# mariusbaehr/gauss_newton_via_generalized_krylov_subspaces

Measured on NVIDIA B200. Metric: gnk_outer_iterations_per_second, higher is better.
Workload: dtype f64

## Files before the change

### gauss_newton_via_generalized_krylov_subspaces_b200/_lib.py

```python
from __future__ import annotations

import ctypes as C
import os

_HERE = os.path.dirname(os.path.abspath(__file__))
LIB_PATH = os.path.join(_HERE, "libgnk_b200.so")

GNK_MAX_BASIS = 256


class Layout(C.Structure):
    _fields_ = [("n_own", C.c_int64), ("off", C.c_int64), ("ld", C.c_int64), ("m", C.c_int32),
                ("rows", C.c_int32), ("halo", C.c_int32), ("has_lo", C.c_int32), ("has_hi", C.c_int32),
                ("pad_", C.c_int32)]


class Bratu(C.Structure):
    _fields_ = [("c_lap", C.c_double), ("c_adv", C.c_double), ("lam", C.c_double)]


class LinOp(C.Structure):
    _fields_ = [("kind", C.c_int32), ("pad_", C.c_int32), ("sign", C.c_double), ("lay", Layout), ("prm", Bratu),
                ("d_expu", C.c_void_p), ("n_res", C.c_int64), ("p", C.c_int64), ("d_rowptr", C.c_void_p),
                ("d_col", C.c_void_p), ("d_val", C.c_void_p), ("d_rowptr_t", C.c_void_p), ("d_col_t", C.c_void_p),
                ("d_val_t", C.c_void_p)]


_P = C.c_void_p
_I = C.c_int
_L = C.c_int64
_D = C.c_double
_LP = C.POINTER(Layout)
_BP = C.POINTER(Bratu)

SIGNATURES = {
    "gnk_abi_version": (_I, []),
    "gnk_last_error": (C.c_char_p, []),
    "gnk_create": (_I, [C.POINTER(_P), _I]),
    "gnk_destroy": (_I, [_P]),
    "gnk_sm_count": (_I, [_P]),
    "gnk_launch_count": (_L, [_P]),
    "gnk_scalars_fetch": (_I, [_P, _P, _I, _P, _P]),
    "gnk_scalars_wait": (_I, [_P]),
    "gnk_bratu_residual": (_I, [_P, _LP, _BP, _P, _P, _P, _P, _I, _P, _P]),
    "gnk_stencil_apply": (_I, [_P, _LP, _BP, _P, _P, _L, _I, _D, _I, _P, _L, _L, _P]),
    "gnk_stencil_normal_diag": (_I, [_P, _LP, _BP, _P, _P, _P]),
    "gnk_combine": (_I, [_P, _LP, _P, _I, _P, _P, _D, _P, _P]),
    "gnk_combine_step": (_I, [_P, _LP, _P, _I, _P, _P, _D, _P, _P, _P, _P]),
    "gnk_norm_stats": (_I, [_P, _LP, _P, _P, _P]),
    "gnk_normalize": (_I, [_P, _LP, _P, _P, _D, _P, _P, _P]),
    "gnk_normalize_halo": (_I, [_P, _LP, _P, _P, _D, _P, _P, _P]),
    "gnk_cgs_dots": (_I, [_P, _LP, _P, _I, _P, _P, _P]),
    "gnk_cgs_update": (_I, [_P, _LP, _P, _I, _P, _P, _P, _P]),
    "gnk_tsqr_ls": (_I, [_P, _P, _L, _L, _I, _P, _D, _P, _P]),
    "gnk_stencil_gram_ls": (_I, [_P, _LP, _BP, _P, _P, _L, _I, _I, _P, _D, _P, _L, _D, _P, _P]),
    "gnk_tsqr_ls_method": (_I, [_P, _I]),
    "gnk_gram_cgls": (_I, [_P, _P, _L, _L, _I, _P, _D, _D, _P, _P]),
    "gnk_spmm_csr": (_I, [_P, _L, _P, _P, _P, _P, _L, _L, _I, _D, _P, _L, _L, _P]),
    "gnk_csr_row_sumsq": (_I, [_P, _L, _P, _P, _P, _P]),
    "gnk_axpby": (_I, [_P, _L, _D, _P, _D, _P, _P, _P]),
    "gnk_dot": (_I, [_P, _L, _P, _P, _P, _P]),
    "gnk_cgls": (_I, [_P, C.POINTER(LinOp), _P, _D, _I, _P, _P, C.POINTER(_L), _P]),
    "gnk_cgls_x0": (_I, [_P, C.POINTER(LinOp), _P, _P, _D, _I, _P, _P, C.POINTER(_L), _P]),
    "gnk_rosenbrock_residual": (_I, [_P, _L, _D, _P, _P, _P]),
    "gnk_rosenbrock_jacobian": (_I, [_P, _L, _D, _P, _P, _P, _P]),
    "gnk_comm_unique_id": (_I, [_P]),
    "gnk_comm_init": (_I, [_P, _P, _I, _I]),
    "gnk_comm_size": (_I, [_P]),
    "gnk_comm_p2p_export": (_I, [_P, _P]),
    "gnk_comm_p2p_attach": (_I, [_P, _P]),
    "gnk_comm_p2p_enabled": (_I, [_P]),
    "gnk_comm_p2p_disable": (_I, [_P]),
    "gnk_comm_fused_reductions": (_I, [_P]),
    "gnk_comm_allreduce": (_I, [_P, _P, _I, _I, _P]),
    "gnk_comm_halo_exchange": (_I, [_P, _LP, _P, _I, _P]),
    "gnk_comm_allgather_owned": (_I, [_P, _LP, _P, _P, C.POINTER(_L), _P]),
}


class GnkError(RuntimeError):
    pass


_lib = None


def load():
    global _lib
# ... 37 lines not shown
```

### gauss_newton_via_generalized_krylov_subspaces_b200/csrc/bratu_stencil.cu

```cuda
#include "common.cuh"

namespace {

constexpr int TPBX = 128;

template <bool VEC>
struct Pair {
  double a, b;
};

template <bool VEC>
__device__ __forceinline__ Pair<VEC> load_pair(const double* p) {
  Pair<VEC> r;
  if (VEC) {
    double2 v = *reinterpret_cast<const double2*>(p);
    r.a = v.x;
    r.b = v.y;
  } else {
    r.a = *p;
    r.b = 0.0;
  }
  return r;
}
template <bool VEC>
// ... 103 lines not shown
  const int rend = min(rbeg + TR, lay.rows);
  const double* vb = in + (int64_t)col * in_ld + lay.off + j0;
  const double* eb_ = expu ? expu + lay.off + j0 : nullptr;
  double* ob = out + (int64_t)col * out_ld + out_off + j0;
  const bool has_l = j0 > 0, has_r = (j0 + W) < m;
  const double d0 = __dadd_rn(4.0 * prm.c_lap, -prm.c_adv);
  const double c_sup = __dadd_rn(-prm.c_lap, prm.c_adv);
  const double cu = transpose ? c_sup : -prm.c_lap;
  const double cd = transpose ? -prm.c_lap : c_sup;
  const double cl = -prm.c_lap;
  Pair<VEC> up = load_pair<VEC>(vb + (int64_t)(rbeg - 1) * m);
  Pair<VEC> mid = load_pair<VEC>(vb + (int64_t)rbeg * m);
#pragma unroll 2
  for (int r = rbeg; r < rend; ++r) {
    const int64_t ro = (int64_t)r * m;
    Pair<VEC> dn = load_pair<VEC>(vb + ro + m);
    const double lf = has_l ? vb[ro - 1] : 0.0;
    const double rt = has_r ? vb[ro + W] : 0.0;
    double dga = d0, dgb = d0;
    if (eb_) {
      Pair<VEC> e = load_pair<VEC>(eb_ + ro);
      dga = __dadd_rn(d0, __dmul_rn(prm.lam, e.a));
      dgb = __dadd_rn(d0, __dmul_rn(prm.lam, e.b));
    }
    const double ra = VEC ? mid.b : rt;
    const double oa = apply_refbits(cu, cl, dga, cd, up.a, lf, mid.a, ra, dn.a);
    const double ob2 = VEC ? apply_refbits(cu, cl, dgb, cd, up.b, mid.a, mid.b, rt, dn.b) : 0.0;
    store_pair<VEC>(ob + ro, sign * oa, sign * ob2);
    up = mid;
    mid = dn;
  }
}

template <bool VEC>
__global__ void __launch_bounds__(TPBX) normal_diag_kernel(gnk_layout lay, gnk_bratu prm,
                                                            const double* __restrict__ expu, int TR,
                                                            double* __restrict__ out) {
  constexpr int W = VEC ? 2 : 1;
  const int m = lay.m;
  const int j0 = W * (blockIdx.x * TPBX + threadIdx.x);
  if (j0 >= m) return;
  const int rbeg = (int)blockIdx.y * TR;
  const int rend = min(rbeg + TR, lay.rows);
  const double d0 = 4.0 * prm.c_lap - prm.c_adv;
  const double cl2 = prm.c_lap * prm.c_lap;
  const double cd2 = (prm.c_adv - prm.c_lap) * (prm.c_adv - prm.c_lap);
  for (int r = rbeg; r < rend; ++r) {
    const int64_t ro = lay.off + (int64_t)r * m + j0;
    double dga = d0, dgb = d0;
    if (expu) {
      Pair<VEC> e = load_pair<VEC>(expu + ro);
      dga = fma(prm.lam, e.a, d0);
      dgb = fma(prm.lam, e.b, d0);
    }
    const bool above = (r > 0) || lay.has_lo;
    const bool below = (r < lay.rows - 1) || lay.has_hi;
    double base = (above ? cd2 : 0.0) + (below ? cl2 : 0.0);
    double a = dga * dga + base + ((j0 > 0) ? cl2 : 0.0) + ((j0 + 1 < m) ? cl2 : 0.0);
    double b = 0.0;
    if (VEC) b = dgb * dgb + base + cl2 + ((j0 + 2 < m) ? cl2 : 0.0);
    store_pair<VEC>(out + ro, a, b);
  }
}


inline int pick_tr(const gnk_ctx* ctx, int gx, int rows, int mult) {
// ... 47 lines not shown
  if (vec)
    GNK_CUDA(gnk_launch(gnk_pdl_for(lay->n_own), residual_kernel<true>, grid, dim3(TPBX), 0, (cudaStream_t)stream, *lay, *prm, d_u, d_y, d_F, d_expu,
                        depth, tr, part, ctx->d_tickets + TK_RESID, d_loss, pd));
  else
    GNK_CUDA(gnk_launch(gnk_pdl_for(lay->n_own), residual_kernel<false>, grid, dim3(TPBX), 0, (cudaStream_t)stream, *lay, *prm, d_u, d_y, d_F,
                        d_expu, depth, tr, part, ctx->d_tickets + TK_RESID, d_loss, pd));
  GNK_LAUNCH_CHECK(ctx);
  return 0;
}

int gnk_stencil_apply(gnk_ctx* ctx, const gnk_layout* lay, const gnk_bratu* prm, const double* d_expu,
                      const double* d_in, int64_t in_ld, int k, double sign, int transpose, double* d_out,
                      int64_t out_ld, int64_t out_off, void* stream) {
  GNK_REQUIRE(ctx && prm && d_in && d_out, "gnk_stencil_apply: null argument");
  GNK_REQUIRE(check_layout(lay) == 0, "gnk_stencil_apply: inconsistent stencil layout");
  GNK_REQUIRE(k >= 1 && k <= 65535, "gnk_stencil_apply: k out of range");
  GNK_REQUIRE(prm->lam == 0.0 || d_expu, "gnk_stencil_apply: e^u diagonal required when lam != 0");
  const bool vec = (lay->m % 2) == 0 && (in_ld % 2) == 0 && (out_ld % 2) == 0 && (out_off % 2) == 0;
  const int gx = (int)ceil_div(lay->m, (vec ? 2 : 1) * TPBX);
  const int tr = pick_tr(ctx, gx, lay->rows, k);
  dim3 grid(k, gx, (unsigned)ceil_div(lay->rows, tr));
  GNK_REQUIRE(grid.z <= 65535, "gnk_stencil_apply: too many row tiles");
  const double* e = (prm->lam == 0.0) ? nullptr : d_expu;
  if (vec)
    GNK_CUDA(gnk_launch(gnk_pdl_for(lay->n_own), apply_kernel<true>, grid, dim3(TPBX), 0, (cudaStream_t)stream, *lay, *prm, e, d_in, in_ld, sign,
                        transpose, tr, d_out, out_ld, out_off));
  else
    GNK_CUDA(gnk_launch(gnk_pdl_for(lay->n_own), apply_kernel<false>, grid, dim3(TPBX), 0, (cudaStream_t)stream, *lay, *prm, e, d_in, in_ld, sign,
                        transpose, tr, d_out, out_ld, out_off));
  GNK_LAUNCH_CHECK(ctx);
  return 0;
}

int gnk_stencil_normal_diag(gnk_ctx* ctx, const gnk_layout* lay, const gnk_bratu* prm, const double* d_expu,
                            double* d_out, void* stream) {
  GNK_REQUIRE(ctx && prm && d_out, "gnk_stencil_normal_diag: null argument");
  GNK_REQUIRE(check_layout(lay) == 0, "gnk_stencil_normal_diag: inconsistent stencil layout");
  GNK_REQUIRE(prm->lam == 0.0 || d_expu, "gnk_stencil_normal_diag: e^u diagonal required when lam != 0");
  const bool vec = (lay->m % 2) == 0;
  const int gx = (int)ceil_div(lay->m, (vec ? 2 : 1) * TPBX);
  const int tr = pick_tr(ctx, gx, lay->rows, 1);
  dim3 grid(gx, (unsigned)ceil_div(lay->rows, tr));
  const double* e = (prm->lam == 0.0) ? nullptr : d_expu;
  if (vec)
    normal_diag_kernel<true><<<grid, TPBX, 0, (cudaStream_t)stream>>>(*lay, *prm, e, tr, d_out);
  else
    normal_diag_kernel<false><<<grid, TPBX, 0, (cudaStream_t)stream>>>(*lay, *prm, e, tr, d_out);
  GNK_LAUNCH_CHECK(ctx);
  return 0;
}

}
```

### gauss_newton_via_generalized_krylov_subspaces_b200/csrc/common.cuh

```cuda
#pragma once
#include <cuda_runtime.h>
#include <stdint.h>
#include <stdio.h>
#include <string>

#include "gnk_b200.h"

struct gnk_ctx {
  int device = 0;
  int sm_count = 148;
  int64_t launches = 0;
  double* d_partials = nullptr;
  unsigned int* d_tickets = nullptr;
  double* d_rbuf[2] = {nullptr, nullptr};
  size_t rbuf_bytes = 0;
  void* nccl_comm = nullptr;
  int rank = 0, nranks = 1;
  double* d_gather = nullptr;
  size_t gather_bytes = 0;
  double* h_pinned = nullptr;
  void* p2p_local = nullptr;
  void* p2p_peer[16] = {nullptr};
  void** d_p2p_peer = nullptr;
  unsigned long long p2p_seq = 0;
  unsigned long long p2p_hseq = 0;
  int p2p_ready = 0;
  int p2p_fused = 0;
  double* d_apart = nullptr;
  size_t apart_bytes = 0;
  double* d_cholqr = nullptr;
  double* d_gramw = nullptr;
  int ls_method = 0;
  cudaStream_t fetch_stream = nullptr;
  cudaEvent_t fetch_event = nullptr;
  cudaEvent_t cg_event[4] = {nullptr, nullptr, nullptr, nullptr};
};
int gnk_ensure_fetch_stream(gnk_ctx* ctx);

constexpr int GNK_PARTIALS = 1 << 19;
constexpr int GNK_TICKETS = 64;

constexpr int64_t PART_STATS = 0;
constexpr int64_t PART_DOTS = 8192;
constexpr int64_t PART_UPDATE = PART_DOTS + 1184 * GNK_MAX_BASIS;
constexpr int64_t PART_DOT1 = PART_UPDATE + 8192;
constexpr int64_t PART_CG = PART_DOT1 + 8192;
constexpr int64_t PART_SCAL = PART_CG + 8192;
constexpr int64_t PART_RESID = GNK_PARTIALS - 65536;
static_assert(PART_SCAL + 64 <= PART_RESID, "partials scratch overflow");

enum TicketSlot { TK_RESID = 0, TK_STATS = 1, TK_DOTS = 2, TK_UPDATE = 3, TK_DOT1 = 4, TK_CG = 5, TK_APPLY_DOTS = 6,
                  TK_CHOLQR = 7, TK_NORMALIZE = 8, TK_GRAMW = 9 };

void gnk_set_error(const std::string& s);
int gnk_fail(const char* what, cudaError_t e, const char* file, int line);

#define GNK_CUDA(expr)                                                    \
  do {                                                                    \
    cudaError_t e__ = (expr);                                             \
    if (e__ != cudaSuccess) return gnk_fail(#expr, e__, __FILE__, __LINE__); \
  } while (0)

#define GNK_LAUNCH_CHECK(ctx)                                             \
  do {                                                                    \
    (ctx)->launches++;                                                    \
    cudaError_t e__ = cudaGetLastError();                                 \
    if (e__ != cudaSuccess) return gnk_fail("kernel launch", e__, __FILE__, __LINE__); \
  } while (0)

#define GNK_REQUIRE(cond, msg)                                            \
  do {                                                                    \
    if (!(cond)) {                                                        \
      gnk_set_error(std::string(msg) + " (" #cond ")");                   \
      return -2;                                                          \
    }                                                                     \
  } while (0)

__device__ __forceinline__ double warp_sum(double v) {
#pragma unroll
  for (int o = 16; o > 0; o >>= 1) v += __shfl_xor_sync(0xffffffffu, v, o);
  return v;
}
__device__ __forceinline__ double warp_max(double v) {
#pragma unroll
  for (int o = 16; o > 0; o >>= 1) v = fmax(v, __shfl_xor_sync(0xffffffffu, v, o));
// ... 117 lines not shown
      asm volatile("ld.volatile.global.v4.u32 {%0, %1, %2, %3}, [%4];" : "=r"(lo), "=r"(t1), "=r"(hi), "=r"(t2) : "l"(p) : "memory");
      if (global_ns() - t0 > P2P_TIMEOUT_NS) __trap();
    } while (t1 != tag || t2 != tag);
  }
  return __hiloint2double((int)hi, (int)lo);
}
__device__ __forceinline__ void p2p_tail_allreduce(const gnk_p2p_dev& pd, double* vals, int count, int op) {
  const int t = threadIdx.x;
  if (t >= count) return;
  const int parity = (int)(pd.seq & 1ull);
  const unsigned tag = (unsigned)(pd.seq % 0xFFFFFFFFull) + 1u;
  const double v = vals[t];
  for (int r = 0; r < pd.nranks; ++r)
    st_ll(static_cast<char*>(pd.peers[r]) + p2p_ll_off(pd.nranks, parity, pd.rank) + 16 * (size_t)t, v, tag);
  const char* mine = static_cast<const char*>(pd.peers[pd.rank]);
  const bool is_max = (op == 1) || (op == 2 && t == 1);
  double a = ld_ll(mine + p2p_ll_off(pd.nranks, parity, 0) + 16 * (size_t)t, tag);
  for (int r = 1; r < pd.nranks; ++r) {
    const double b = ld_ll(mine + p2p_ll_off(pd.nranks, parity, r) + 16 * (size_t)t, tag);
    a = is_max ? fmax(a, b) : a + b;
  }
  vals[t] = a;
}

__device__ __forceinline__ double apply_refbits(double cu, double cl, double dg, double cd, double up, double lf,
                                                double mid, double rt, double dn) {
  double s = __dadd_rn(__dmul_rn(cu, up), __dmul_rn(cl, lf));
  s = __dadd_rn(s, __dmul_rn(dg, mid));
  s = __dadd_rn(s, __dmul_rn(cl, rt));
  s = __dadd_rn(s, __dmul_rn(cd, dn));
  return s;
}

static inline int64_t ceil_div(int64_t a, int64_t b) { return (a + b - 1) / b; }

__device__ __forceinline__ void pdl_begin() {
  asm volatile("griddepcontrol.wait;" ::: "memory");
  asm volatile("griddepcontrol.launch_dependents;" ::: "memory");
}
int gnk_pdl_mode();
constexpr int64_t GNK_PDL_MAX_N = 6 * 1024 * 1024;
inline bool gnk_pdl_for(int64_t n_unknowns) {
  const int mode = gnk_pdl_mode();
  return mode == 2 || (mode == 1 && n_unknowns <= GNK_PDL_MAX_N);
}
template <typename... P, typename... A>
inline cudaError_t gnk_launch(bool pdl, void (*kern)(P...), dim3 grid, dim3 block, size_t smem, cudaStream_t st,
                              A&&... args) {
  cudaLaunchConfig_t cfg = {};
  cfg.gridDim = grid;
  cfg.blockDim = block;
  cfg.dynamicSmemBytes = smem;
  cfg.stream = st;
  cudaLaunchAttribute at[1];
  at[0].id = cudaLaunchAttributeProgrammaticStreamSerialization;
  at[0].val.programmaticStreamSerializationAllowed = pdl ? 1 : 0;
  cfg.attrs = at;
  cfg.numAttrs = 1;
  return cudaLaunchKernelEx(&cfg, kern, static_cast<P>(args)...);
}
```

### gauss_newton_via_generalized_krylov_subspaces_b200/csrc/vector_ops.cu

```cuda
#include "common.cuh"

namespace {

constexpr int TPB = 256;

__device__ __forceinline__ double2 ld2(const double* p) { return *reinterpret_cast<const double2*>(p); }
__device__ __forceinline__ double2 ld2_stream(const double* p) {
  return __ldcs(reinterpret_cast<const double2*>(p));
}
__device__ __forceinline__ void st2(double* p, double2 v) { *reinterpret_cast<double2*>(p) = v; }

__global__ void __launch_bounds__(TPB) combine_kernel(const double* __restrict__ V, int64_t ld, int64_t len,
                                                       int k, const double* __restrict__ c,
                                                       const double* __restrict__ d, double s,
                                                       double* __restrict__ x, double* __restrict__ c_out,
                                                       double* __restrict__ cprev2) {
  __shared__ double coef[GNK_MAX_BASIS];
  pdl_begin();
  for (int j = threadIdx.x; j < k; j += blockDim.x) coef[j] = d ? (c[j] + s * d[j]) : c[j];
  __syncthreads();
  if (blockIdx.x == 0) {
    if (c_out) {
      for (int j = threadIdx.x; j <= k && j < GNK_MAX_BASIS; j += blockDim.x) c_out[j] = (j < k) ? coef[j] : 0.0;
    }
    if (cprev2 && threadIdx.x < 32) {
      double a = 0.0;
      for (int j = threadIdx.x; j < k; j += 32) a = fma(c[j], c[j], a);
      a = warp_sum(a);
      if (threadIdx.x == 0) cprev2[0] = a;
    }
  }
  const int64_t nv = len >> 1;
  const int64_t stride = (int64_t)gridDim.x * blockDim.x;
  for (int64_t i = (int64_t)blockIdx.x * blockDim.x + threadIdx.x; i < nv; i += stride) {
    const double* p = V + 2 * i;
    double2 acc = make_double2(0.0, 0.0);
    int j = 0;
    for (; j + 8 <= k; j += 8) {
      double2 v[8];
#pragma unroll
      for (int u = 0; u < 8; ++u) v[u] = ld2_stream(p + (int64_t)(j + u) * ld);
#pragma unroll
      for (int u = 0; u < 8; ++u) {
        acc.x = fma(v[u].x, coef[j + u], acc.x);
        acc.y = fma(v[u].y, coef[j + u], acc.y);
      }
    }
    for (; j < k; ++j) {
      double2 v = ld2_stream(p + (int64_t)j * ld);
      acc.x = fma(v.x, coef[j], acc.x);
      acc.y = fma(v.y, coef[j], acc.y);
    }
    st2(x + 2 * i, acc);
  }
}

__global__ void __launch_bounds__(TPB) stats_kernel(const double* __restrict__ x, int64_t n,
                                                     double* __restrict__ partials, unsigned int* ticket,
                                                     double* __restrict__ out) {
  __shared__ double sh[32];
  const int64_t nv = n >> 1;
  const int64_t gt = (int64_t)blockIdx.x * blockDim.x + threadIdx.x;
  const int64_t stride = (int64_t)gridDim.x * blockDim.x;
  double ss = 0.0, mx = 0.0;
// ... 418 lines not shown
```

### gauss_newton_via_generalized_krylov_subspaces_b200/gauss_newton_krylow.py

```python
from __future__ import annotations

import ctypes as C
import os
import weakref
from typing import Any, Callable, Optional, Tuple

import numpy as np

from . import _lib
from .armijo_goldstein import armijo_device
from .bratu_pde_problem import BratuDeviceProblem
from .device import DeviceVector, HostCallableProblem, get_runtime, make_layout, ptr
from .krylow import (GeneralizedKrylowSubspace, GeneralizedKrylowSubspaceBreakdown,
                     GeneralizedKrylowSubspaceSpansEntireSpace, MAX_COLUMNS)
from .partition import flat_layout_fields, round_up, tensor_ls_on_every_rank
from .regression_result import RegressionResult
from .rosenbrock_problem import RosenbrockDeviceProblem

_NB = _lib.GNK_MAX_BASIS
_SC_LOSS = 2 * _NB + 8
_SC_CPREV = _SC_LOSS + 2
_SC_FLAG = _SC_CPREV + 2
_SC_FLAG2 = _SC_CPREV + 3
_BLK = _SC_CPREV + 6
# ... 192 lines not shown
        r0 = np.asarray(res(prob.download_global(x_trial), *args), dtype=np.float64).reshape(-1)
        prob._ensure_res_layout(r0.shape[0])
    F_cur, F_trial = prob.new_res(), prob.new_res()
    res_off = prob.res_fields["off"]
    n_res_own = prob.res_fields["n_own"]
    ldjv = round_up(max(n_res_own, 1), 16)
    use_aux = is_bratu and prob.pb.LAMBDA != 0
    aux = [prob.new_sol() for _ in range(3)] if use_aux else [None, None, None]
    hx = prob.d.halo_exchange if (is_bratu and prob.distributed) else None
    ls_method = 0
    if is_bratu and prob.distributed and not tensor_ls_on_every_rank(prob.sol_fields["m"], rt.world):
        ls_method = 1

    if native:
        prob.residual(x_trial, F_cur, loss_slot, aux=None)
    else:
        rt.upload(r0, F_cur[:n_res_own])
        prob.sumsq(F_cur, loss_slot, prob.res_lay)
    nfev = 1
    prev_loss = float(rt.read(loss_slot, 1)[0])
    jac_ev = prob.jacobian(x_start, aux=None)
    if use_aux:
        aux[0] = jac_ev.expu
    njev = 1

    JV = None
    jv_cap = 0
    state = {"pending": False, "fslot": _SC_FLAG}

    def other_slot():
        return _SC_FLAG2 if state["fslot"] == _SC_FLAG else _SC_FLAG

    defer_ok = ls_solver == "qr" and os.environ.get("GNK_DEFER_BREAKDOWN", "1") != "0"

    for iter in range(1, max_iter):
        for attempt in (0, 1):
            k = krylow.k
            state["rank_reported"] = False
            if k > jv_cap:
                jv_cap = min(MAX_COLUMNS, max(krylow.cap, k))
                JV = rt.empty(jv_cap * ldjv)
            ls_done = False
            if (is_bratu and ls_solver == "qr" and ls_method == 0 and not jac_ev.transposed
                    and jac_ev.scale == 1.0):
                with rt.mark("spmm+ls", 8.0 * n_res_own * (3 * k + 2)) as mk:
                    rc = lib.gnk_stencil_gram_ls(rt.ctx, C.byref(sol_lay), C.byref(prob.d.prm), ptr(jac_ev.expu),
                                                 ptr(krylow.V), ld, krylow.cap, k, ptr(F_cur), -1.0, ptr(JV), ldjv,
                                                 -1.0, ptr(blk), rt.stream)
                    mk.cancel = rc != 0
                if rc == 0:
                    ls_done = True
                elif rc != 1:
                    _lib.check(rc, "gnk_stencil_gram_ls")
            if not ls_done:
                with rt.mark("spmm", 8.0 * n_res_own * (2 * k + 1)):
                    jac_ev.matmat(krylow.V, ld, k, JV, ldjv)
            if ls_done:
                pass
            elif ls_solver == "qr":
                with rt.mark("tsqr", 8.0 * n_res_own * (k + 1)):
                    tsqr_solve(rt, JV, ldjv, n_res_own, k, F_cur[res_off:], -1.0, blk, method=ls_method)
            elif ls_solver == "cgls":
                if k + 1 <= 56 and n_res_own % 2 == 0 and ldjv % 2 == 0:
                    with rt.mark("gram_cgls", 8.0 * n_res_own * (k + 1)):
                        _lib.check(lib.gnk_gram_cgls(rt.ctx, ptr(JV), ldjv, n_res_own, k, ptr(F_cur, res_off), -1.0,
                                                     float(cg_rtol), ptr(blk), rt.stream), "gnk_gram_cgls")
                else:
                    cgls_dense(rt, JV, ldjv, n_res_own, k, F_cur[res_off:], -1.0, cg_rtol, blk)
            else:
                raise ValueError("ls_solver must be 'qr' or 'cgls'")
            spec_ok = (native and defer_ok and iter + 1 < max_iter and iter % krylow_restart != 0
                       and version in _VERSIONS and krylow.k < prob.p_glob
                       and os.environ.get("GNK_SPECULATE", "1") != "0")
            state["spec"] = None

            def expansion_operands(jac_new):
                if version == "res_old":
                    return jac_new, F_cur
                if version == "res_new":
                    return jac_new, F_trial
                if version == "jac_old_res_old":
                    return jac_ev, F_cur
                return jac_ev, F_trial

            def trial_loss(s):
                krylow.dev_combine(c, blk, s, x_trial, c_out=c_next, cprev2=ptr(blk, _SC_CPREV))
                with rt.mark("residual", 32.0 * n_res_own):
                    prob.residual(x_trial, F_trial, loss_slot, aux=aux[1])
                if spec_ok and state["spec"] is None:
                    pending_read = rt.read_begin(blk, _BLK)
                    jac_new = prob.jacobian(x_trial, aux=aux[1])
                    krylow.dev_expand_enqueue(*expansion_operands(jac_new), hx, ptr(blk, other_slot()))
                    state["spec"] = jac_new
                    state["vals"] = rt.read_end(pending_read)
                else:
                    if state["spec"] is not None:
                        state["spec"] = False
                    state["vals"] = rt.read(blk, _BLK)
                if state["pending"] and state["vals"][state["fslot"]:state["fslot"] + 1].view(np.int32)[0] != 0:
                    raise _DeferredBreakdown()
                if ls_solver == "qr" and ls_refused(state["vals"], k):
                    raise _LeastSquaresRefused()
                if ls_solver == "qr" and not state["rank_reported"]:
                    state["rank_reported"] = True
                    _report_rank(state["vals"], k)
                return float(state["vals"][_SC_LOSS])

            def line_search():
                return armijo_device(trial_loss, prev_loss, lambda: float(state["vals"][k]),
                                     lambda: float(np.sqrt(state["vals"][k + 3])))

            try:
                step_length, nfev_delta = line_search()
            except _DeferredBreakdown:
                state["pending"] = False
                krylow.retract()
                print(f"Generalized krylow subspace breakdown at iteration = {iter - 1}, "
                      f"basis.shape = ({prob.p_glob}, {krylow.k})")
                continue
            except _LeastSquaresRefused:
                with rt.mark("tsqr", 8.0 * n_res_own * (k + 1)):
                    tsqr_solve(rt, JV, ldjv, n_res_own, k, F_cur[res_off:], -1.0, blk, householder=True)
                state["rank_reported"] = False
                step_length, nfev_delta = line_search()
            state["pending"] = False
# ... 69 lines not shown
```

### gauss_newton_via_generalized_krylov_subspaces_b200/krylow.py

```python
from __future__ import annotations

import ctypes as C
import math

import numpy as np

from . import _lib
from .device import CsrJacobian, HostCallableProblem, get_runtime, make_layout, ptr
from .partition import flat_layout_fields

MAX_COLUMNS = _lib.GNK_MAX_BASIS - 1


class GeneralizedKrylowSubspaceBreakdown(Exception):
    pass


class GeneralizedKrylowSubspaceSpansEntireSpace(Exception):
    pass


class _FlatOwner:

    def __init__(self, rt, n):
# ... 28 lines not shown
        self.flag = rt.zeros(1, dtype=rt.torch.int32)
        self._ready = True

    def _grow(self):
        if self.cap >= MAX_COLUMNS:
            raise _lib.GnkError(f"Krylov basis wider than {MAX_COLUMNS} columns is not supported; pass krylow_restart")
        new_cap = min(MAX_COLUMNS, max(self.cap * 2, 2), self.n_glob)
        V = self.rt.empty(new_cap * self.ld)
        V[:self.k * self.ld].copy_(self.V[:self.k * self.ld])
        self.V, self.cap = V, new_cap

    def col(self, j):
        return self.V[j * self.ld:(j + 1) * self.ld]

    def dev_start(self, x):
        rt, lib = self.rt, self.rt.lib
        _lib.check(lib.gnk_norm_stats(rt.ctx, C.byref(self.lay), ptr(x), ptr(self.stats), rt.stream), "gnk_norm_stats")
        rt.allreduce(self.stats, 2, 2)
        _lib.check(lib.gnk_normalize(rt.ctx, C.byref(self.lay), ptr(x), ptr(self.stats), 1e-8, ptr(self.V),
                                     ptr(self.flag), rt.stream), "gnk_normalize")
        ss = rt.read(self.stats, 2)
        if ss[1] <= 1e-8:
            raise ValueError("x0 is not allowed to be 0 in the gauss_newton_krylow algorithm")
        self.k = 1
        return math.sqrt(ss[0])

    def dev_combine(self, c, d, s, out, c_out=None, cprev2=None):
        rt = self.rt
        with rt.mark("combine", 8.0 * self.fields["n_own"] * (self.k + 1)):
            _lib.check(rt.lib.gnk_combine_step(rt.ctx, C.byref(self.lay), ptr(self.V), self.k, ptr(c), ptr(d), float(s),
                                               ptr(out), ptr(c_out), cprev2 if cprev2 is not None else ptr(None),
                                               rt.stream), "gnk_combine")

    def dev_expand_enqueue(self, jac_op, r, halo_exchange=None, flag_ptr=None):
        if self.k == self.n_glob:
            raise GeneralizedKrylowSubspaceSpansEntireSpace
        rt, lib = self.rt, self.rt.lib
        if self.k == self.cap:
            self._grow()
        n = self.fields["n_own"]
        with rt.mark("spmv_t", 24.0 * n):
            jac_op.neg_rmatvec(r, self.w)
        for ipass in range(self.reorth_passes):
            with rt.mark("cgs_dots", 8.0 * n * (self.k + 1)):
                _lib.check(lib.gnk_cgs_dots(rt.ctx, C.byref(self.lay), ptr(self.V), self.k, ptr(self.w),
                                            ptr(self.h), rt.stream), "gnk_cgs_dots")
            if not rt.fused_reductions:
                rt.allreduce(self.h, self.k, 0)
            with rt.mark("cgs_update", 8.0 * n * (self.k + 2)):
                _lib.check(lib.gnk_cgs_update(rt.ctx, C.byref(self.lay), ptr(self.V), self.k, ptr(self.h),
                                              ptr(self.w), ptr(self.stats), rt.stream), "gnk_cgs_update")
        if not rt.fused_reductions:
            rt.allreduce(self.stats, 2, 2)
        new = self.col(self.k)
        fp = ptr(self.flag) if flag_ptr is None else flag_ptr
        with rt.mark("normalize", 16.0 * n):
            if halo_exchange is not None:
                _lib.check(lib.gnk_normalize_halo(rt.ctx, C.byref(self.lay), ptr(self.w), ptr(self.stats), 1e-8,
                                                  ptr(new), fp, rt.stream), "gnk_normalize_halo")
            else:
                _lib.check(lib.gnk_normalize(rt.ctx, C.byref(self.lay), ptr(self.w), ptr(self.stats), 1e-8, ptr(new),
                                             fp, rt.stream), "gnk_normalize")

    def commit(self):
        self.k += 1

    def dev_update(self, jac_op, r, halo_exchange=None, deferred_flag=None):
        self.dev_expand_enqueue(jac_op, r, halo_exchange, deferred_flag)
        if deferred_flag is None and int(self.rt.read_i32(self.flag)[0]) != 0:
            raise GeneralizedKrylowSubspaceBreakdown(
                "Normal residual is allready inside generalized Krylow Subspcae, there for gauss newton krylow "
                "algorithm has to proceed without enlarging the subspace.")
        self.commit()

    def retract(self):
        self.k -= 1

    @property
    def basis(self):
        cols = [self.owner.download_global(self.col(j)) for j in range(self.k)]
        return np.stack(cols, axis=1)
# ... 47 lines not shown
```

### include/gnk_b200.h

```cpp
#ifndef GNK_B200_H
#define GNK_B200_H

#include <stdint.h>

#ifdef __cplusplus
extern "C" {
#endif

#define GNK_B200_ABI_VERSION 1
#define GNK_MAX_BASIS 256
#define GNK_TSQR_MAX 104

typedef struct gnk_ctx gnk_ctx;

typedef struct {
  int64_t n_own;
  int64_t off;
  int64_t ld;
  int32_t m;
  int32_t rows;
  int32_t halo;
  int32_t has_lo;
  int32_t has_hi;
  int32_t pad_;
// ... 7 lines not shown

int gnk_abi_version(void);
const char* gnk_last_error(void);
int gnk_create(gnk_ctx** out, int device);
int gnk_destroy(gnk_ctx* ctx);
int gnk_sm_count(gnk_ctx* ctx);
int64_t gnk_launch_count(gnk_ctx* ctx);
int gnk_scalars_fetch(gnk_ctx* ctx, const double* d_src, int count, double* h_dst, void* stream);
int gnk_scalars_wait(gnk_ctx* ctx);

int gnk_bratu_residual(gnk_ctx* ctx, const gnk_layout* lay, const gnk_bratu* prm, const double* d_u,
                       const double* d_y, double* d_F, double* d_expu, int depth, double* d_loss,
                       void* stream);
int gnk_stencil_apply(gnk_ctx* ctx, const gnk_layout* lay, const gnk_bratu* prm, const double* d_expu,
                      const double* d_in, int64_t in_ld, int k, double sign, int transpose,
                      double* d_out, int64_t out_ld, int64_t out_off, void* stream);
int gnk_stencil_normal_diag(gnk_ctx* ctx, const gnk_layout* lay, const gnk_bratu* prm,
                            const double* d_expu, double* d_out, void* stream);

int gnk_combine(gnk_ctx* ctx, const gnk_layout* lay, const double* d_V, int k, const double* d_c,
                const double* d_d, double s, double* d_x, void* stream);
int gnk_combine_step(gnk_ctx* ctx, const gnk_layout* lay, const double* d_V, int k, const double* d_c,
                     const double* d_d, double s, double* d_x, double* d_c_out, double* d_cprev2, void* stream);
int gnk_norm_stats(gnk_ctx* ctx, const gnk_layout* lay, const double* d_x, double* d_stats, void* stream);
int gnk_normalize(gnk_ctx* ctx, const gnk_layout* lay, const double* d_x, const double* d_stats,
                  double atol, double* d_out, int32_t* d_flag, void* stream);
int gnk_normalize_halo(gnk_ctx* ctx, const gnk_layout* lay, const double* d_x, const double* d_stats, double atol,
                       double* d_out, int32_t* d_flag, void* stream);
int gnk_cgs_dots(gnk_ctx* ctx, const gnk_layout* lay, const double* d_V, int k, const double* d_w,
                 double* d_h, void* stream);
int gnk_cgs_update(gnk_ctx* ctx, const gnk_layout* lay, const double* d_V, int k, const double* d_h,
                   double* d_w, double* d_stats, void* stream);

int gnk_tsqr_ls(gnk_ctx* ctx, const double* d_A, int64_t lda, int64_t n_rows, int k,
                const double* d_y, double sign_a, double* d_out, void* stream);

int gnk_stencil_gram_ls(gnk_ctx* ctx, const gnk_layout* lay, const gnk_bratu* prm, const double* d_expu,
                        const double* d_V, int64_t ldv, int v_cols, int k, const double* d_r, double sign,
                        double* d_JV, int64_t ldjv, double sign_a, double* d_out, void* stream);

int gnk_tsqr_ls_method(gnk_ctx* ctx, int method);

int gnk_spmm_csr(gnk_ctx* ctx, int64_t n_rows, const int32_t* d_rowptr, const int32_t* d_col,
                 const double* d_val, const double* d_in, int64_t in_ld, int64_t in_off, int k,
                 double sign, double* d_out, int64_t out_ld, int64_t out_off, void* stream);
int gnk_csr_row_sumsq(gnk_ctx* ctx, int64_t n_rows, const int32_t* d_rowptr, const double* d_val,
                      double* d_out, void* stream);

int gnk_axpby(gnk_ctx* ctx, int64_t n, double a, const double* d_x, double b, const double* d_y,
              double* d_out, void* stream);
int gnk_dot(gnk_ctx* ctx, int64_t n, const double* d_x, const double* d_y, double* d_out, void* stream);

typedef struct {
  int32_t kind;
  int32_t pad_;
  double sign;
  gnk_layout lay;
  gnk_bratu prm;
  const double* d_expu;
  int64_t n_res, p;
  const int32_t *d_rowptr, *d_col;
  const double* d_val;
  const int32_t *d_rowptr_t, *d_col_t;
  const double* d_val_t;
} gnk_linop;
int gnk_cgls(gnk_ctx* ctx, const gnk_linop* op, const double* d_y, double rtol, int preconditioner,
// ... 29 lines not shown
```

Before: 361.5.

## Fuse trial combine, Bratu residual, transpose apply and CGS dots into one kernel

Adds a single streaming kernel that, for the speculative trial step, forms x = V·coef, evaluates the Bratu residual and e^u, applies the transposed Jacobian to the current residual to produce w, and accumulates the first-pass CGS dot products and the loss via a grid-wide last-block reduction. The Python driver uses it for single-rank Bratu runs when k is between 4 and 31 and skips the separate spmv_t and first cgs_dots launches. The goal is to read V once instead of several times and to cut kernel launches. The cost is a complex kernel with high register use for larger KB, extra halo-row recomputation, and a fallback path when its conditions are not met.

```diff
diff --git a/gauss_newton_via_generalized_krylov_subspaces_b200/_lib.py b/gauss_newton_via_generalized_krylov_subspaces_b200/_lib.py
--- a/gauss_newton_via_generalized_krylov_subspaces_b200/_lib.py
+++ b/gauss_newton_via_generalized_krylov_subspaces_b200/_lib.py
@@ -54,6 +54,7 @@
     "gnk_cgs_update": (_I, [_P, _LP, _P, _I, _P, _P, _P, _P]),
     "gnk_tsqr_ls": (_I, [_P, _P, _L, _L, _I, _P, _D, _P, _P]),
     "gnk_stencil_gram_ls": (_I, [_P, _LP, _BP, _P, _P, _L, _I, _I, _P, _D, _P, _L, _D, _P, _P]),
+    "gnk_bratu_trial_expand": (_I, [_P, _LP, _BP, _P, _I, _P, _P, _D, _P, _P, _P, _P, _P, _P, _P, _P, _P, _P, _P]),
     "gnk_tsqr_ls_method": (_I, [_P, _I]),
     "gnk_gram_cgls": (_I, [_P, _P, _L, _L, _I, _P, _D, _D, _P, _P]),
     "gnk_spmm_csr": (_I, [_P, _L, _P, _P, _P, _P, _L, _L, _I, _D, _P, _L, _L, _P]),
diff --git a/gauss_newton_via_generalized_krylov_subspaces_b200/csrc/bratu_stencil.cu b/gauss_newton_via_generalized_krylov_subspaces_b200/csrc/bratu_stencil.cu
--- a/gauss_newton_via_generalized_krylov_subspaces_b200/csrc/bratu_stencil.cu
+++ b/gauss_newton_via_generalized_krylov_subspaces_b200/csrc/bratu_stencil.cu
@@ -159,6 +159,154 @@
   }
 }
 
+constexpr int TRIAL_EXPAND_MIN_K = 4;
+
+struct TrialExpand {
+  gnk_layout lay;
+  gnk_bratu prm;
+  const double* V;
+  const double* c;
+  const double* d;
+  double s;
+  int k, TR;
+  const double* y;
+  const double* Fc;
+  double *x, *F, *expu, *w, *c_out, *cprev2;
+  double* partials;
+  unsigned int* ticket;
+  double *h, *loss;
+};
+
+template <int KB, int NW>
+__global__ void __launch_bounds__(32 * NW, KB <= 8 ? 3 : (KB <= 16 ? 2 : 1)) trial_expand_kernel(const TrialExpand a) {
+  constexpr int TE_TJ = 32 * (NW - 1), TE_NT = 32 * NW;
+  __shared__ double coef[KB];
+  __shared__ double xs[4][TE_TJ + 2];
+  __shared__ double wpart[NW][32];
+  pdl_begin();
+  const bool first_cta = blockIdx.x == 0 && blockIdx.y == 0;
+  combine_coefficients(a.c, a.d, a.s, a.k, coef, first_cta, a.c_out, a.cprev2);
+  const gnk_layout& L = a.lay;
+  const gnk_bratu& prm = a.prm;
+  const int m = L.m, k = a.k, tid = threadIdx.x;
+  const int64_t ld = L.ld;
+  if (first_cta) {
+    const int64_t e = (int64_t)(L.rows + 2 * L.halo) * m + tid;
+    if (e < ld) {
+      double xv = 0.0;
+      for (int j = 0; j < k; ++j) xv = fma(a.V[(int64_t)j * ld + e], coef[j], xv);
+      a.x[e] = xv;
+    }
+  }
+  const int j0 = (int)blockIdx.x * TE_TJ;
+  const bool edge = tid >= TE_TJ;
+  const int jc = !edge ? j0 + tid : (tid == TE_TJ ? j0 - 1 : (tid == TE_TJ + 1 ? j0 + TE_TJ : -1));
+  const int slot = !edge ? tid + 1 : (tid == TE_TJ ? 0 : (tid == TE_TJ + 1 ? TE_TJ + 1 : -1));
+  const bool live = jc >= 0 && jc < m;
+  const bool own = !edge && live;
+  const bool has_l = jc > 0, has_r = jc + 1 < m;
+  const int q0 = -1 + (int)blockIdx.y * a.TR, q1 = min(q0 + a.TR, L.rows + 1);
+  const int64_t pc = L.off + (live ? jc : 0);
+  const double* Vp = a.V + pc;
+  const double c4 = 4.0 * prm.c_lap;
+  const double d0 = __dadd_rn(4.0 * prm.c_lap, -prm.c_adv);
+  const double cu = __dadd_rn(-prm.c_lap, prm.c_adv), cl = -prm.c_lap, cd = -prm.c_lap;
+
+  double v[KB], hacc[KB];
+#pragma unroll
+  for (int j = 0; j < KB; ++j) hacc[j] = 0.0;
+  double lacc = 0.0;
+  auto load_v = [&](int r) {
+    const int64_t ro = (int64_t)r * m;
+#pragma unroll
+    for (int j = 0; j < KB; ++j)
+      if (j < k && live) v[j] = __ldcs(Vp + (int64_t)j * ld + ro);
+  };
+  auto load_fc = [&](int r) { return (own && r >= -2 && r <= L.rows + 1) ? a.Fc[pc + (int64_t)r * m] : 0.0; };
+  double fu = load_fc(q0 - 2), fm = load_fc(q0 - 1), fd, fl, fr;
+  auto load_step = [&](int r) {
+    load_v(r);
+    fd = load_fc(r + 1);
+    const bool wrow = own && r >= 0 && r < L.rows;
+    fl = (wrow && has_l) ? a.Fc[pc + (int64_t)r * m - 1] : 0.0;
+    fr = (wrow && has_r) ? a.Fc[pc + (int64_t)r * m + 1] : 0.0;
+  };
+  load_step(q0 - 1);
+  double e_prev = 1.0;
+  for (int r = q0 - 1; r <= q1; ++r) {
+    const int64_t ro = (int64_t)r * m;
+    double xr = 0.0;
+#pragma unroll
+    for (int j = 0; j < KB; ++j)
+      if (j < k && live) xr = fma(v[j], coef[j], xr);
+    double er = 1.0;
+    if (prm.lam != 0.0) er = exp(xr);
+    if (own && ((r >= q0 && r < q1) || r == -2 || r == L.rows + 1)) a.x[pc + ro] = xr;
+    if (own && r >= q0 && r < q1 && r >= 0 && r < L.rows) {
+      const double dg = (prm.lam != 0.0) ? __dadd_rn(d0, __dmul_rn(prm.lam, er)) : d0;
+      const double wv = apply_refbits(cu, cl, dg, cd, fu, fl, fm, fr, fd);
+      a.w[pc + ro] = wv;
+#pragma unroll
+      for (int j = 0; j < KB; ++j)
+        if (j < k) hacc[j] = fma(v[j], wv, hacc[j]);
+    }
+    if (slot >= 0) xs[(r + 4) & 3][slot] = xr;
+    fu = fm;
+    fm = fd;
+    const int q = r - 1;
+    const bool frow = own && q >= q0;
+    const double yv = frow ? a.y[pc + (int64_t)q * m] : 0.0;
+    if (r < q1) load_step(r + 1);
+    __syncthreads();
+    if (frow) {
+      const double* xu = xs[(q + 3) & 3];
+      const double* xm = xs[(q + 4) & 3];
+      const double* xd = xs[(r + 4) & 3];
+      double p = pde_refbits(prm, c4, xu[slot], xm[slot - 1], xm[slot], xm[slot + 1], xd[slot]);
+      if (prm.lam != 0.0) p = __dadd_rn(p, __dmul_rn(prm.lam, e_prev));
+      double f = __dsub_rn(yv, p);
+      const bool owned = q >= 0 && q < L.rows;
+      if (!(owned || (q < 0 ? L.has_lo : L.has_hi))) f = 0.0;
+      a.F[pc + (int64_t)q * m] = f;
+      if (a.expu) a.expu[pc + (int64_t)q * m] = e_prev;
+      if (owned) lacc = fma(f, f, lacc);
+    }
+    e_prev = er;
+  }
+
+  const int lane = tid & 31, wid = tid >> 5;
+#pragma unroll
+  for (int j = 0; j < KB; ++j) {
+    if (j < k) {
+      const double r = warp_sum(hacc[j]);
+      if (lane == 0) wpart[wid][j] = r;
+    }
+  }
+  {
+    const double r = warp_sum(lacc);
+    if (lane == 0) wpart[wid][31] = r;
+  }
+  __syncthreads();
+  const unsigned int bid = linear_block_id();
+  if (tid < 32 && (tid < k || tid == 31)) {
+    double r = wpart[0][tid];
+#pragma unroll
+    for (int q = 1; q < NW; ++q) r += wpart[q][tid];
+    a.partials[(int64_t)bid * 32 + tid] = r;
+    __threadfence();
+  }
+  if (grid_arrive_last(a.ticket)) {
+    const int nb = (int)total_blocks();
+    for (int j = wid; j < 32; j += NW) {
+      if (j >= k && j != 31) continue;
+      double s = 0.0;
+      for (int b = lane; b < nb; b += 32) s += __ldcg(a.partials + (int64_t)b * 32 + j);
+      s = warp_sum(s);
+      if (lane == 0) (j == 31 ? a.loss[0] : a.h[j]) = s;
+    }
+  }
+}
+
 template <bool VEC>
 __global__ void __launch_bounds__(TPBX) normal_diag_kernel(gnk_layout lay, gnk_bratu prm,
                                                             const double* __restrict__ expu, int TR,
@@ -272,6 +420,58 @@
   return 0;
 }
 
+}
+
+namespace {
+
+template <int KB, int NW>
+int launch_trial_expand(gnk_ctx* ctx, TrialExpand& a, cudaStream_t st) {
+  auto kern = trial_expand_kernel<KB, NW>;
+  static int per_sm[64] = {0};
+  int& ps = per_sm[ctx->device & 63];
+  if (ps == 0) GNK_CUDA(cudaOccupancyMaxActiveBlocksPerMultiprocessor(&ps, kern, 32 * NW, 0));
+  const int gx = (int)ceil_div(a.lay.m, 32 * (NW - 1));
+  const int frows = a.lay.rows + 2;
+  int64_t strips = (int64_t)(ps > 0 ? ps : 1) * ctx->sm_count / gx;
+  if (strips < 1) strips = 1;
+  if (strips > frows) strips = frows;
+  a.TR = (int)ceil_div(frows, strips);
+  dim3 grid(gx, (unsigned)ceil_div(frows, a.TR));
+  GNK_REQUIRE((int64_t)grid.x * grid.y <= 1184, "gnk_bratu_trial_expand: grid exceeds the partials scratch");
+  GNK_CUDA(gnk_launch(gnk_pdl_for(a.lay.n_own), kern, grid, dim3(32 * NW), 0, st, a));
+  GNK_LAUNCH_CHECK(ctx);
+  return 0;
+}
+
+}
+
+extern "C" {
+
+int gnk_bratu_trial_expand(gnk_ctx* ctx, const gnk_layout* lay, const gnk_bratu* prm, const double* d_V, int k,
+                           const double* d_c, const double* d_d, double s, const double* d_y, const double* d_Fcur,
+                           double* d_x, double* d_F, double* d_expu, double* d_w, double* d_c_out, double* d_cprev2,
+                           double* d_h, double* d_loss, void* stream) {
+  GNK_REQUIRE(ctx && lay && prm && d_V && d_c && d_y && d_Fcur && d_x && d_F && d_w && d_h && d_loss,
+              "gnk_bratu_trial_expand: null argument");
+  GNK_REQUIRE(lay->m > 0 && lay->rows > 0 && lay->halo == 2 && lay->off == 2LL * lay->m &&
+                  lay->n_own == (int64_t)lay->rows * lay->m && lay->ld >= (int64_t)(lay->rows + 4) * lay->m,
+              "gnk_bratu_trial_expand: inconsistent stencil layout");
+  GNK_REQUIRE(k >= 1, "gnk_bratu_trial_expand: k out of range");
+  GNK_REQUIRE(d_c_out != d_c, "gnk_bratu_trial_expand: c_out must not alias c (rejected trials re-read c)");
+  const bool aligned = (lay->ld % 2 == 0) && ((uintptr_t)d_V % 16 == 0) && ((uintptr_t)d_y % 16 == 0) &&
+                       ((uintptr_t)d_Fcur % 16 == 0) && ((uintptr_t)d_x % 16 == 0) && ((uintptr_t)d_F % 16 == 0) &&
+                       ((uintptr_t)d_w % 16 == 0) && (d_expu == nullptr || (uintptr_t)d_expu % 16 == 0);
+  if (!(ctx->nranks == 1 && lay->m % 8 == 0 && lay->n_own >= 16384 && aligned && k <= 31 && k >= TRIAL_EXPAND_MIN_K))
+    return 1;
+  TrialExpand a{*lay, *prm, d_V, d_c, d_d, s, k, 0, d_y, d_Fcur, d_x, d_F, d_expu, d_w, d_c_out, d_cprev2,
+                ctx->d_partials + PART_TRIAL, ctx->d_tickets + TK_TRIAL, d_h, d_loss};
+  cudaStream_t st = (cudaStream_t)stream;
+  if (k <= 8) return launch_trial_expand<8, 8>(ctx, a, st);
+  if (k <= 16) return launch_trial_expand<16, 8>(ctx, a, st);
+  if (k <= 24) return launch_trial_expand<24, 12>(ctx, a, st);
+  return launch_trial_expand<32, 8>(ctx, a, st);
+}
+
 int gnk_stencil_normal_diag(gnk_ctx* ctx, const gnk_layout* lay, const gnk_bratu* prm, const double* d_expu,
                             double* d_out, void* stream) {
   GNK_REQUIRE(ctx && prm && d_out, "gnk_stencil_normal_diag: null argument");
diff --git a/gauss_newton_via_generalized_krylov_subspaces_b200/csrc/common.cuh b/gauss_newton_via_generalized_krylov_subspaces_b200/csrc/common.cuh
--- a/gauss_newton_via_generalized_krylov_subspaces_b200/csrc/common.cuh
+++ b/gauss_newton_via_generalized_krylov_subspaces_b200/csrc/common.cuh
@@ -46,11 +46,12 @@
 constexpr int64_t PART_DOT1 = PART_UPDATE + 8192;
 constexpr int64_t PART_CG = PART_DOT1 + 8192;
 constexpr int64_t PART_SCAL = PART_CG + 8192;
+constexpr int64_t PART_TRIAL = PART_SCAL + 64;
 constexpr int64_t PART_RESID = GNK_PARTIALS - 65536;
-static_assert(PART_SCAL + 64 <= PART_RESID, "partials scratch overflow");
+static_assert(PART_TRIAL + 1184 * 32 <= PART_RESID, "partials scratch overflow");
 
 enum TicketSlot { TK_RESID = 0, TK_STATS = 1, TK_DOTS = 2, TK_UPDATE = 3, TK_DOT1 = 4, TK_CG = 5, TK_APPLY_DOTS = 6,
-                  TK_CHOLQR = 7, TK_NORMALIZE = 8, TK_GRAMW = 9 };
+                  TK_CHOLQR = 7, TK_NORMALIZE = 8, TK_GRAMW = 9, TK_TRIAL = 10 };
 
 void gnk_set_error(const std::string& s);
 int gnk_fail(const char* what, cudaError_t e, const char* file, int line);
@@ -234,6 +235,24 @@
   return s;
 }
 
+__device__ __forceinline__ void combine_coefficients(const double* __restrict__ c, const double* __restrict__ d,
+                                                     double s, int k, double* coef, bool writer,
+                                                     double* __restrict__ c_out, double* __restrict__ cprev2) {
+  for (int j = threadIdx.x; j < k; j += blockDim.x) coef[j] = d ? (c[j] + s * d[j]) : c[j];
+  __syncthreads();
+  if (writer) {
+    if (c_out) {
+      for (int j = threadIdx.x; j <= k && j < GNK_MAX_BASIS; j += blockDim.x) c_out[j] = (j < k) ? coef[j] : 0.0;
+    }
+    if (cprev2 && threadIdx.x < 32) {
+      double a = 0.0;
+      for (int j = threadIdx.x; j < k; j += 32) a = fma(c[j], c[j], a);
+      a = warp_sum(a);
+      if (threadIdx.x == 0) cprev2[0] = a;
+    }
+  }
+}
+
 static inline int64_t ceil_div(int64_t a, int64_t b) { return (a + b - 1) / b; }
 
 __device__ __forceinline__ void pdl_begin() {
diff --git a/gauss_newton_via_generalized_krylov_subspaces_b200/csrc/vector_ops.cu b/gauss_newton_via_generalized_krylov_subspaces_b200/csrc/vector_ops.cu
--- a/gauss_newton_via_generalized_krylov_subspaces_b200/csrc/vector_ops.cu
+++ b/gauss_newton_via_generalized_krylov_subspaces_b200/csrc/vector_ops.cu
@@ -17,19 +17,7 @@
                                                        double* __restrict__ cprev2) {
   __shared__ double coef[GNK_MAX_BASIS];
   pdl_begin();
-  for (int j = threadIdx.x; j < k; j += blockDim.x) coef[j] = d ? (c[j] + s * d[j]) : c[j];
-  __syncthreads();
-  if (blockIdx.x == 0) {
-    if (c_out) {
-      for (int j = threadIdx.x; j <= k && j < GNK_MAX_BASIS; j += blockDim.x) c_out[j] = (j < k) ? coef[j] : 0.0;
-    }
-    if (cprev2 && threadIdx.x < 32) {
-      double a = 0.0;
-      for (int j = threadIdx.x; j < k; j += 32) a = fma(c[j], c[j], a);
-      a = warp_sum(a);
-      if (threadIdx.x == 0) cprev2[0] = a;
-    }
-  }
+  combine_coefficients(c, d, s, k, coef, blockIdx.x == 0, c_out, cprev2);
   const int64_t nv = len >> 1;
   const int64_t stride = (int64_t)gridDim.x * blockDim.x;
   for (int64_t i = (int64_t)blockIdx.x * blockDim.x + threadIdx.x; i < nv; i += stride) {
diff --git a/gauss_newton_via_generalized_krylov_subspaces_b200/gauss_newton_krylow.py b/gauss_newton_via_generalized_krylov_subspaces_b200/gauss_newton_krylow.py
--- a/gauss_newton_via_generalized_krylov_subspaces_b200/gauss_newton_krylow.py
+++ b/gauss_newton_via_generalized_krylov_subspaces_b200/gauss_newton_krylow.py
@@ -248,6 +248,8 @@
         return _SC_FLAG2 if state["fslot"] == _SC_FLAG else _SC_FLAG
 
     defer_ok = ls_solver == "qr" and os.environ.get("GNK_DEFER_BREAKDOWN", "1") != "0"
+    trial_fused = (is_bratu and rt.world == 1 and version == "res_old" and hasattr(lib, "gnk_bratu_trial_expand")
+                   and os.environ.get("GNK_TRIAL_FUSED", "1") != "0")
 
     for iter in range(1, max_iter):
         for attempt in (0, 1):
@@ -300,13 +302,18 @@
                 return jac_ev, F_trial
 
             def trial_loss(s):
-                krylow.dev_combine(c, blk, s, x_trial, c_out=c_next, cprev2=ptr(blk, _SC_CPREV))
-                with rt.mark("residual", 32.0 * n_res_own):
-                    prob.residual(x_trial, F_trial, loss_slot, aux=aux[1])
-                if spec_ok and state["spec"] is None:
+                speculate = spec_ok and state["spec"] is None
+                fused = speculate and trial_fused and krylow.dev_trial_expand(
+                    c, blk, s, x_trial, c_next, ptr(blk, _SC_CPREV), prob.d.prm, prob.res.y_col, F_cur, F_trial,
+                    aux[1], loss_slot)
+                if not fused:
+                    krylow.dev_combine(c, blk, s, x_trial, c_out=c_next, cprev2=ptr(blk, _SC_CPREV))
+                    with rt.mark("residual", 32.0 * n_res_own):
+                        prob.residual(x_trial, F_trial, loss_slot, aux=aux[1])
+                if speculate:
                     pending_read = rt.read_begin(blk, _BLK)
                     jac_new = prob.jacobian(x_trial, aux=aux[1])
-                    krylow.dev_expand_enqueue(*expansion_operands(jac_new), hx, ptr(blk, other_slot()))
+                    krylow.dev_expand_enqueue(*expansion_operands(jac_new), hx, ptr(blk, other_slot()), w_ready=fused)
                     state["spec"] = jac_new
                     state["vals"] = rt.read_end(pending_read)
                 else:
diff --git a/gauss_newton_via_generalized_krylov_subspaces_b200/krylow.py b/gauss_newton_via_generalized_krylov_subspaces_b200/krylow.py
--- a/gauss_newton_via_generalized_krylov_subspaces_b200/krylow.py
+++ b/gauss_newton_via_generalized_krylov_subspaces_b200/krylow.py
@@ -84,21 +84,38 @@
                                                ptr(out), ptr(c_out), cprev2 if cprev2 is not None else ptr(None),
                                                rt.stream), "gnk_combine")
 
-    def dev_expand_enqueue(self, jac_op, r, halo_exchange=None, flag_ptr=None):
+    def dev_trial_expand(self, c, d, s, out, c_out, cprev2, prm, y, F_cur, F, expu, loss_slot):
+        rt = self.rt
+        if self.k == self.cap:
+            self._grow()
+        n = self.fields["n_own"]
+        with rt.mark("trial_expand", 8.0 * n * self.k + 48.0 * n) as mk:
+            rc = rt.lib.gnk_bratu_trial_expand(rt.ctx, C.byref(self.lay), C.byref(prm), ptr(self.V), self.k, ptr(c),
+                                               ptr(d), float(s), ptr(y), ptr(F_cur), ptr(out), ptr(F), ptr(expu),
+                                               ptr(self.w), ptr(c_out), cprev2, ptr(self.h), ptr(loss_slot),
+                                               rt.stream)
+            mk.cancel = rc != 0
+        if rc not in (0, 1):
+            _lib.check(rc, "gnk_bratu_trial_expand")
+        return rc == 0
+
+    def dev_expand_enqueue(self, jac_op, r, halo_exchange=None, flag_ptr=None, w_ready=False):
         if self.k == self.n_glob:
             raise GeneralizedKrylowSubspaceSpansEntireSpace
         rt, lib = self.rt, self.rt.lib
         if self.k == self.cap:
             self._grow()
         n = self.fields["n_own"]
-        with rt.mark("spmv_t", 24.0 * n):
-            jac_op.neg_rmatvec(r, self.w)
+        if not w_ready:
+            with rt.mark("spmv_t", 24.0 * n):
+                jac_op.neg_rmatvec(r, self.w)
         for ipass in range(self.reorth_passes):
-            with rt.mark("cgs_dots", 8.0 * n * (self.k + 1)):
-                _lib.check(lib.gnk_cgs_dots(rt.ctx, C.byref(self.lay), ptr(self.V), self.k, ptr(self.w),
-                                            ptr(self.h), rt.stream), "gnk_cgs_dots")
-            if not rt.fused_reductions:
-                rt.allreduce(self.h, self.k, 0)
+            if ipass > 0 or not w_ready:
+                with rt.mark("cgs_dots", 8.0 * n * (self.k + 1)):
+                    _lib.check(lib.gnk_cgs_dots(rt.ctx, C.byref(self.lay), ptr(self.V), self.k, ptr(self.w),
+                                                ptr(self.h), rt.stream), "gnk_cgs_dots")
+                if not rt.fused_reductions:
+                    rt.allreduce(self.h, self.k, 0)
             with rt.mark("cgs_update", 8.0 * n * (self.k + 2)):
                 _lib.check(lib.gnk_cgs_update(rt.ctx, C.byref(self.lay), ptr(self.V), self.k, ptr(self.h),
                                               ptr(self.w), ptr(self.stats), rt.stream), "gnk_cgs_update")
diff --git a/include/gnk_b200.h b/include/gnk_b200.h
--- a/include/gnk_b200.h
+++ b/include/gnk_b200.h
@@ -63,6 +63,11 @@
 int gnk_cgs_update(gnk_ctx* ctx, const gnk_layout* lay, const double* d_V, int k, const double* d_h,
                    double* d_w, double* d_stats, void* stream);
 
+int gnk_bratu_trial_expand(gnk_ctx* ctx, const gnk_layout* lay, const gnk_bratu* prm, const double* d_V, int k,
+                           const double* d_c, const double* d_d, double s, const double* d_y, const double* d_Fcur,
+                           double* d_x, double* d_F, double* d_expu, double* d_w, double* d_c_out, double* d_cprev2,
+                           double* d_h, double* d_loss, void* stream);
+
 int gnk_tsqr_ls(gnk_ctx* ctx, const double* d_A, int64_t lda, int64_t n_rows, int k,
                 const double* d_y, double sign_a, double* d_out, void* stream);
 
```

New measurement: 368.9 (median of 6 runs). 2.1% higher.
